# nbip/IWAE

Hardware: AMD Instinct MI355X
Metric: images/sec (train step) IWAE k=50 batch 1024 @1/2/4/8 GPU; test LLH@k=5000 (higher is better)
Workload: dtype bf16; 1 GPU; 1-layer IWAE k=50 batch 1024 per GPU (BASELINE configs[1]; N=8 is configs[4]), objective iwae_elbo, train step = forward + backward + Adam(eps=1e-4); config_id=c1, global_batch=1024, n_samples=50, parallelism=dp1, rccl_ranks=0, settle_steps=100, full=False

## Files before the change

iwae_amd/csrc/kernels.h:

```cpp
#pragma once
#include <hip/hip_runtime.h>
#include <stdint.h>

namespace iwae {

#define IWAE_DENSE_G1_DEFAULT 29u
enum { EPI_TANH = 0, EPI_HEAD = 1, EPI_DX = 2, EPI_F32 = 3, EPI_BERN = 4, EPI_SIGMOID = 5 };
enum { OBJ_VAE_ELBO = 0, OBJ_IWAE_ELBO = 1, OBJ_IWAE_EQ14 = 2, OBJ_VAE_ELBO_KL = 3, OBJ_DREG = 4 };
enum { PB_LME = 0, PB_MEAN, PB_EQ14, PB_KL, PB_PX, PB_T1, PB_T2, PB_DREG, PB_COUNT };
enum { SC_VAE_ELBO = 0, SC_VAE_ELBO_KL, SC_IWAE_ELBO, SC_IWAE_EQ14, SC_INFERENCE_LOSS, SC_MEAN_LPXZ, SC_MEAN_T1, SC_MEAN_T2, SC_KL, SC_COUNT = 16 };

struct EpsSrc {
    const float* user = nullptr;
    const float* cache = nullptr;
    int ldC = 0;
    int B = 0;
    uint64_t seed = 0;
    uint64_t row_offset = 0;
    uint32_t step = 0;
    uint32_t stream = 0;
    int k_total = 0, s_off = 0, kc = 0;
};

struct LseArgs {
// ... 4 lines not shown
    const float* head; int ldH, D, Dp;
    float* logw; float* wn; float* gx; float4* cf; float* per_b;
    int n_px_part; size_t px_stride;
    float* term0_out;
    int lme_only;
    float* gx_local; int gx_r0, gx_n;
};

struct DenseArgs {
    const uint16_t* X; int ldX;
    const char* img;
    int split;
    int M, KT, MG, mg_per_block;
    int stage_all;
    unsigned g1_mask;
    int Np32;
    uint16_t* YP; int ldYP;
    float* YF; int ldYF;
    const uint16_t* ACT; int ldACT;
    const uint16_t* XB; int ldXB; int k; int B; int Xdim;
    const float* zhead; int ldZH;
    const float* zeps; int zldE; int zD, zDp;
    uint16_t* ZPout;
    float* zlp; float* zlq;
    float* zlq_dreg;
    float* lpxz; size_t lpxz_stride;
    float* logits_out;
    int pipe;
    const char* pre_img1; int pre_KT1;
    const char* pre_img2;
    const uint16_t* pre_Z;
    uint16_t *pre_G1, *pre_G2;
    unsigned long long* stamps;
    int lse_on;
    LseArgs lse;
    uint16_t* G2W; int g2w_feat;
    int dbg;
};

struct SampleArgs {
    const float* head; int ldH; int Dp; int D; int head_per_row;
    int M, Mp, k, B;
    EpsSrc eps;
    uint16_t* ZP;
    float* ZF; int ldZF;
    const float* prior_head;
    const float* cond; int C;
    float* lp_prior; float* lq; float* lq_dreg;
};

struct BlockFwdArgs {
    const uint16_t* X; int ldX;
    const float* Xf; int Xdim; uint16_t* XPout;
    const char *img0, *img1, *img2;
    int KT0, KT1;
    int NT1, NT2;
    int R;
    uint16_t *H1, *H2; int ldH;
    float* YF; int ldYF; int split;
    int sample; SampleArgs S;
    const char* oimg; int oXdim, oH;
    const uint16_t* oXB; int oldXB; int ok;
    uint16_t* oSP; int oldS; float* olpxz;
};
struct DecBwdRowsArgs {
    const uint16_t* SP; int ldS; int KTX;
// ... 343 lines not shown
```

iwae_amd/csrc/kernels.hip:

```cpp
#include <hip/hip_runtime.h>
#include <hip/hip_ext.h>
#include <stdint.h>
#include <string.h>
#include <type_traits>
#include <algorithm>
#include "kernels.h"
#include "layout.h"

#ifdef IWAE_DIAG
#define WG_DBG(a, bit) (((a).dbg & (bit)) != 0)
#else
#define WG_DBG(a, bit) false
#endif
namespace iwae {

typedef __attribute__((ext_vector_type(8))) __bf16 bf16x8_t;
typedef __attribute__((ext_vector_type(2))) __bf16 bf16x2_t;
typedef __attribute__((ext_vector_type(4))) float f32x4;

#define LOG2PI_F 1.8378770664093453f

__device__ __forceinline__ uint32_t pack2(float a, float b) {
    bf16x2_t v;
    v[0] = (__bf16)a;
// ... 160 lines not shown
template <bool MASKED, bool KEEP>
__device__ __forceinline__ float bern8(const f32x4& a0, const f32x4& a1, const uint4& xb, int f0, int Xdim, uint4& sp) {
    float s_xl = 0.0f, s_al = 0.0f, prod = 1.0f, sv[8];
#pragma unroll
    for (int j = 0; j < 8; ++j) {
        const float l = (j < 4) ? a0[j & 3] : a1[j & 3];
        const float xm = bf_at(xb, j) - 0.5f;
        const float ope = 1.0f + exp2_raw(-fabsf(l * LOG2E_F));
        const bool in = !MASKED || (f0 + 16 * (j >> 2) + (j & 3) < Xdim);
        prod *= in ? ope : 1.0f;
        s_al += fabsf(l);
        s_xl = fmaf(xm, l, s_xl);
        if (KEEP) {
            const float h = __builtin_copysignf(rcp_fast(ope) - 0.5f, l);
            sv[j] = in ? xm - h : 0.0f;
        }
    }
    if (KEEP) sp = make_uint4(pack2(sv[0], sv[1]), pack2(sv[2], sv[3]), pack2(sv[4], sv[5]), pack2(sv[6], sv[7]));
    return s_xl - 0.5f * s_al - LN2_F * log2_raw(prod);
}

#define DENSE_UNIT 33792

#ifdef IWAE_DENSE_STAMPS
#define DS_STAMP(slot)                                                                 \
    {                                                                                  \
        unsigned long long t_;                                                         \
        __builtin_amdgcn_sched_barrier(0);                                             \
        asm volatile("s_memtime %0\n\ts_waitcnt lgkmcnt(0)" : "=s"(t_)::"memory");     \
        __builtin_amdgcn_sched_barrier(0);                                             \
        ds_sum[slot] += t_ - ds_prev;                                                  \
        ds_prev = t_;                                                                  \
    }
#else
#define DS_STAMP(slot)
#endif

template <int EPI, int KTC, int G, int NWV = (G == 2 ? 4 : 8), bool ZIN = false>
__global__ __launch_bounds__(64 * NWV, G == 1 ? 4 : ((EPI == EPI_BERN && KTC > 0) ? 2 : 1)) void dense_kernel(DenseArgs a) {
#ifdef IWAE_DENSE_STAMPS
    unsigned long long ds_sum[8] = {0, 0, 0, 0, 0, 0, 0, 0}, ds_prev = 0;
    asm volatile("s_memtime %0\n\ts_waitcnt lgkmcnt(0)" : "=s"(ds_prev)::"memory");
#endif
    extern __shared__ __attribute__((aligned(1024))) char smem[];
    const int lane = threadIdx.x & 63, wave = __builtin_amdgcn_readfirstlane(threadIdx.x >> 6);
    const int rho = lane & 15, q = lane >> 4;
    const int r0 = (blockIdx.x * NWV + wave) * (16 * G);
    int row[G], rowc[G];
    bool valid[G];
#pragma unroll
    for (int g = 0; g < G; ++g) { row[g] = r0 + G * rho + g; valid[g] = row[g] < a.M; rowc[g] = min(row[g], a.M - 1); }
    const int a_off = rho * 64 + ((q ^ hperm(rho >> 2)) * 16);
    const int KT = KTC ? KTC : a.KT;
    const int nkw = KTC ? 1 : ((KT + 7) >> 3);
    const int mg0 = blockIdx.y * a.mg_per_block;
    const int mg1 = min(a.MG, mg0 + a.mg_per_block);
    const int nunits = (mg1 - mg0) * nkw;
    const size_t gbytes = img_mg_group_bytes(KT);
    constexpr bool kPacked = (EPI == EPI_TANH || EPI == EPI_DX);
    constexpr bool kPre = (EPI == EPI_DX || EPI == EPI_BERN);
    constexpr bool kBiasInit = (EPI == EPI_BERN) && KTC > 0;

    uint4 bfr[8][G];
    auto load_b_into = [&](int kw, uint4 (&dst)[8][G]) {
#pragma unroll
        for (int ks = 0; ks < 8; ++ks) {
#pragma unroll
            for (int g = 0; g < G; ++g) {
// ... 895 lines not shown
    if (has) {
        const uint2 v = valid ? dtanh(acc, y2, gxr) : make_uint2(0, 0);
        *(uint2*)(act1 + kso * 1024 + a_off + 8 * hh) = v;
        if (valid) *(uint2*)(a.D2P + (size_t)row * a.ldH + kso * 32 + q * 8 + 4 * hh) = v;
    }
    __syncthreads();
    acc = (f32x4){0.f, 0.f, 0.f, 0.f};
#pragma unroll
    for (int ks = 0; ks < BLOCKFWD_MAX_KT; ++ks)
        if (ks < a.KT) acc = mfma16(A2[ks], *(const uint4*)(act1 + ks * 1024 + a_off), acc);
    if (has) {
        const uint2 v = valid ? dtanh(acc, y1, 1.0f) : make_uint2(0, 0);
        *(uint2*)(act2 + kso * 1024 + a_off + 8 * hh) = v;
        if (valid) *(uint2*)(a.D1P + (size_t)row * a.ldH + kso * 32 + q * 8 + 4 * hh) = v;
    }
    __syncthreads();
    acc = (f32x4){0.f, 0.f, 0.f, 0.f};
#pragma unroll
    for (int ks = 0; ks < BLOCKFWD_MAX_KT; ++ks)
        if (ks < a.KT) acc = mfma16(A1[ks], *(const uint4*)(act2 + ks * 1024 + a_off), acc);
    if (has3 && valid) {
        const int f0 = 16 * wave + 4 * q;
        if (a.DZH) *(uint2*)(a.DZH + (size_t)row * a.ldDZ + f0) = make_uint2(pack2(acc[0], acc[1]), pack2(acc[2], acc[3]));
        else *(float4*)(a.DZ + (size_t)row * a.ldDZ + f0) = make_float4(acc[0], acc[1], acc[2], acc[3]);
    }
}

#define BERN_XIMG_MAX 5
template <int KTC, bool KEEP, bool PRE, bool QW = false>
__global__ __launch_bounds__(QW ? 1024 : 512, 4) void bern_pipe_kernel(DenseArgs a) {
#ifdef IWAE_DENSE_STAMPS
    unsigned long long ds_sum[8] = {0, 0, 0, 0, 0, 0, 0, 0}, ds_prev = 0;
    asm volatile("s_memtime %0\n\ts_waitcnt lgkmcnt(0)" : "=s"(ds_prev)::"memory");
#endif
    extern __shared__ __attribute__((aligned(1024))) char smem[];
    constexpr int NWV = QW ? 16 : 8, ROWS = QW ? 200 : 128;
    constexpr int UNIT = KTC * 4096 + 1024, NPC = 4 * KTC + 1, NIDX = (NPC + NWV - 1) / NWV, NF = 2 * KTC, P = 4;
    const int lane = threadIdx.x & 63, wave = __builtin_amdgcn_readfirstlane(threadIdx.x >> 6);
    const int rho = lane & 15, q = lane >> 4;
    const int tile = QW ? min(wave, 12) : wave;
    const int qw = QW ? wave - 12 : -1;
    const int row = blockIdx.x * ROWS + tile * 16 + rho;
    const bool valid = row < a.M && tile * 16 + rho < ROWS;
    const bool storer = qw <= 0;
    if (QW && qw >= 0) __builtin_amdgcn_s_setprio(3);
    const int rowc = min(row, a.M - 1);
    const int a_off = rho * 64 + ((q ^ hperm(rho >> 2)) * 16);
    const int H = a.Np32 >> 5;
    const size_t gbytes = img_mg_group_bytes(KTC);

    auto dma_group = [&](int g, int buf) {
#pragma unroll
        for (int idx = 0; idx < NIDX; ++idx) {
            const int p = wave + NWV * idx;
            if (p < NPC)
                glds16(a.img + (size_t)g * gbytes + (size_t)p * 1024 + lane * 16,
                       (uint32_t)__builtin_amdgcn_readfirstlane((int)(lds_addr_of(smem + buf * UNIT) + (uint32_t)p * 1024u)));
        }
    };
    constexpr int MGH = (2 * KTC + 3) / 4;
    auto dma_unit = [&](int u, int buf) {
        const char* src = a.img;
        int npc = NPC;
        if (u < MGH) { src = a.pre_img1 + (size_t)u * img_mg_group_bytes(a.pre_KT1); npc = 4 * a.pre_KT1 + 1; }
        else if (u < 2 * MGH) src = a.pre_img2 + (size_t)(u - MGH) * gbytes;
        if (WG_DBG(a, 64) && u < 2 * MGH) return;
#pragma unroll
        for (int idx = 0; idx < NIDX; ++idx) {
            const int p = wave + NWV * idx;
            if (p < npc)
                glds16(src + (size_t)p * 1024 + lane * 16,
                       (uint32_t)__builtin_amdgcn_readfirstlane((int)(lds_addr_of(smem + buf * UNIT) + (uint32_t)p * 1024u)));
        }
    };
    if constexpr (PRE) dma_unit(0, 0);
    else dma_group(0, 0);
    char* lx = smem + 2 * UNIT;
    const int blk_r0 = blockIdx.x * ROWS;
    const int b0 = blk_r0 / a.k, b1 = min(blk_r0 + ROWS - 1, a.M - 1) / a.k;
    constexpr bool ZQ = PRE && QW;
    constexpr int HZ_OFF = 2 * UNIT + 128 + 4096 + 2 * KTC * 1024 + 4096 + 1024;
    float4 ze[8];
    if constexpr (PRE) {
        if (a.zhead) {
            const float* er = a.zeps + (size_t)rowc * a.zldE;
            const int flast = a.zldE - 4;
#pragma unroll
            for (int i = 0; i < 8; ++i) ze[i] = *(const float4*)(er + min(32 * (i >> 1) + 16 * (i & 1) + 4 * q, flast));
        }
    }
    if constexpr (ZQ) {
        if (a.zhead) {
            float* hzf = (float*)(smem + HZ_OFF + (size_t)8 * a.ldXB * 4);
            const int zDp = a.zDp, c4 = zDp >> 2, nimg = b1 - b0 + 1;
            for (int o = threadIdx.x; o < nimg * 2 * c4; o += 64 * NWV) {
                const int img = o / (2 * c4), r = o - img * 2 * c4, arr = r >= c4 ? 1 : 0, c = r - arr * c4;
                const float4 v = *(const float4*)(a.zhead + (size_t)(b0 + img) * a.ldZH + arr * zDp + 4 * c);
                float w[4] = {v.x, v.y, v.z, v.w};
#pragma unroll
                for (int i = 0; i < 4; ++i) w[i] = (4 * c + i < a.zD) ? w[i] : 0.0f;
                *(float4*)(hzf + (size_t)(img * 3 + arr) * zDp + 4 * c) = make_float4(w[0], w[1], w[2], w[3]);
            }
        }
    }
    const int xchunks = (b1 - b0 + 1) * a.ldXB / 8;
    for (int o = threadIdx.x; o < xchunks; o += 64 * NWV) {
        const uint4 v = *(const uint4*)(a.XB + (size_t)b0 * a.ldXB + (size_t)o * 8);
        float4 lo, hi;
        lo.x = bflo(v.x) - 0.5f; lo.y = bfhi(v.x) - 0.5f; lo.z = bflo(v.y) - 0.5f; lo.w = bfhi(v.y) - 0.5f;
        hi.x = bflo(v.z) - 0.5f; hi.y = bfhi(v.z) - 0.5f; hi.z = bflo(v.w) - 0.5f; hi.w = bfhi(v.w) - 0.5f;
        *(float4*)(lx + (size_t)o * 32) = lo;
        *(float4*)(lx + (size_t)o * 32 + 16) = hi;
    }
    const char* lxrow = lx + (size_t)(rowc / a.k - b0) * a.ldXB * 4 + q * 32;
    uint4 bfr[KTC];
    if constexpr (!PRE) {
#pragma unroll
        for (int ks = 0; ks < KTC; ++ks) {
            const uint4 v = *(const uint4*)(a.X + (size_t)rowc * a.ldX + ks * 32 + q * 8);
            bfr[ks] = valid ? v : make_uint4(0, 0, 0, 0);
        }
    } else {
        const int KT1 = a.pre_KT1, ldZ = 32 * KT1;
        uint4 zf[4];
        if (a.zhead) {
            const int zDp = a.zDp;
            const int bimg = min(rowc / a.k, b1);
            const bool dreg = a.zlq_dreg != nullptr;
            auto logsig = [&](const float* sgp, float& s1, float& s2) {
                s1 = 0.0f; s2 = 0.0f;
                for (int d = lane; d < a.zD; d += 64) {
                    const float sg = sgp[d];
                    s1 += log2_raw(sg);
                    if (dreg) s2 += log2_raw(sg + 1e-6f);
                }
                s1 = LN2_F * wave_sum(s1); s2 = LN2_F * wave_sum(s2);
            };
            float hs1 = 0.0f, hs2 = 0.0f;
            const float* hm;
            if constexpr (ZQ) {
                float* hzf = (float*)(smem + HZ_OFF + (size_t)8 * a.ldXB * 4);
                float* hsum = hzf + 8 * 3 * zDp;
                __syncthreads();
                if (wave <= b1 - b0) {
                    float s1, s2;
                    logsig(hzf + (size_t)(wave * 3 + 1) * zDp, s1, s2);
                    if (lane == 0) { hsum[2 * wave] = s1; hsum[2 * wave + 1] = s2; }
                }
                __syncthreads();
                hm = hzf + (size_t)(bimg - b0) * 3 * zDp;
                hs1 = hsum[2 * (bimg - b0)]; hs2 = hsum[2 * (bimg - b0) + 1];
            } else {
                hm = a.zhead + (size_t)bimg * a.ldZH;
                const int ilo = __builtin_amdgcn_readlane(bimg, 0), ihi = __builtin_amdgcn_readlane(bimg, 15);
                float s1, s2;
                logsig(a.zhead + (size_t)ilo * a.ldZH + zDp, s1, s2);
                hs1 = s1; hs2 = s2;
                if (ihi != ilo) {
                    logsig(a.zhead + (size_t)ihi * a.ldZH + zDp, s1, s2);
                    if (bimg != ilo) { hs1 = s1; hs2 = s2; }
                }
            }
            float sz = 0.0f, se = 0.0f, su = 0.0f;
#pragma unroll
            for (int ks = 0; ks < 4; ++ks) {
                zf[ks] = make_uint4(0, 0, 0, 0);
                if (ks < KT1) {
                    float z8[8];
#pragma unroll
                    for (int h = 0; h < 2; ++h) {
                        const int f0 = 32 * ks + 16 * h + 4 * q;
                        const float4 mu4 = *(const float4*)(hm + f0), sg4 = *(const float4*)(hm + zDp + f0);
                        const float4 e4 = ze[2 * ks + h];
                        float ev[4] = {e4.x, e4.y, e4.z, e4.w}, muv[4] = {mu4.x, mu4.y, mu4.z, mu4.w};
                        const float sgv[4] = {sg4.x, sg4.y, sg4.z, sg4.w};
                        if (32 * ks + 16 * h + 16 > a.zD) {
#pragma unroll
                            for (int i = 0; i < 4; ++i) { const bool in = f0 + i < a.zD; ev[i] = in ? ev[i] : 0.0f; muv[i] = in ? muv[i] : 0.0f; }
                        }
#pragma unroll
                        for (int i = 0; i < 4; ++i) {
                            const float z = fmaf(sgv[i], ev[i], muv[i]);
                            sz = fmaf(z, z, sz);
                            se = fmaf(ev[i], ev[i], se);
                            z8[4 * h + i] = z;
                        }
                        if (dreg) {
#pragma unroll
                            for (int i = 0; i < 4; ++i) {
                                const float u2 = (sgv[i] * __builtin_amdgcn_rcpf(sgv[i] + 1e-6f)) * ev[i];
                                su = fmaf(u2, u2, su);
                            }
                        }
                    }
                    const uint4 frag = make_uint4(pack2(z8[0], z8[1]), pack2(z8[2], z8[3]), pack2(z8[4], z8[5]), pack2(z8[6], z8[7]));
                    zf[ks] = valid ? frag : make_uint4(0, 0, 0, 0);
                    if (valid && storer && a.ZPout) *(uint4*)(a.ZPout + (size_t)row * ldZ + ks * 32 + q * 8) = frag;
                }
            }
            sz += __shfl_xor(sz, 16); sz += __shfl_xor(sz, 32);
            se += __shfl_xor(se, 16); se += __shfl_xor(se, 32);
            su += __shfl_xor(su, 16); su += __shfl_xor(su, 32);
            const float cD = 0.5f * LOG2PI_F * (float)a.zD;
            const float lp = -0.5f * sz - cD, lq = -0.5f * se - cD - hs1, lq2 = -0.5f * su - cD - hs2;
            if (q == 0 && valid && storer) { a.zlp[row] = lp; a.zlq[row] = lq; if (dreg) a.zlq_dreg[row] = lq2; }
            if constexpr (QW) {
                if (a.lse_on && q == 0 && storer) {
                    float* lz = (float*)(smem + 2 * UNIT + (size_t)8 * a.ldXB * 4 + 128 + 4096 + 2 * KTC * 1024);
                    lz[tile * 16 + rho] = lp; lz[208 + tile * 16 + rho] = lq; lz[416 + tile * 16 + rho] = lq2;
                }
            }
        } else {
#pragma unroll
            for (int ks = 0; ks < 4; ++ks) {
                zf[ks] = make_uint4(0, 0, 0, 0);
                if (ks < KT1) {
                    const uint4 v = *(const uint4*)(a.pre_Z + (size_t)rowc * ldZ + ks * 32 + q * 8);
                    zf[ks] = valid ? v : make_uint4(0, 0, 0, 0);
                }
            }
        }
        uint4 g1f[KTC];
        auto store_group = [&](uint16_t* Gout, const uint4 (&bout)[KTC], int mg) {
            if (!(valid && storer && Gout) || (QW && qw >= 0)) return;
#pragma unroll
            for (int p2 = 0; p2 < 2; ++p2)
                if (2 * mg + p2 < KTC) *(uint4*)(Gout + (size_t)row * (32 * KTC) + (2 * mg + p2) * 32 + q * 8) = bout[2 * mg + p2];
        };
        auto hidden = [&](auto nb_tag, uint4* bin, auto KTin, int ubase, uint4 (&bout)[KTC], uint16_t* Gout, const char* xch_in, char* xch_out, auto&& first) {
            constexpr int NB = decltype(nb_tag)::value;
            const bool quarter = QW && qw >= 0;
#pragma unroll
            for (int mg = 0; mg < MGH; ++mg) {
                const int u = ubase + mg, buf = u & 1;
                wait_all_vmem();
                __syncthreads();
                dma_unit(u + 1, buf ^ 1);
                if (mg == 0) first(); else store_group(Gout, bout, mg - 1);
                const char* lb = smem + buf * UNIT + a_off;
                const char* lbias = smem + buf * UNIT + KTin * 4096 + q * 16;
                if (quarter) {
                    if (mg == 0 && xch_in) {
#pragma unroll
                        for (int ks = 0; ks < NB; ++ks) bin[ks] = *(const uint4*)(xch_in + ks * 1024 + lane * 16);
                    }
                    const float4 c = *(const float4*)(lbias + 64 * qw);
                    f32x4 acc1 = (f32x4){c.x, c.y, c.z, c.w};
#pragma unroll
                    for (int ks = 0; ks < NB; ++ks)
                        if (ks < KTin) acc1 = mfma16(*(const uint4*)(lb + (ks * 4 + qw) * 1024), bin[ks], acc1);
                    const int ft = 4 * mg + qw, kso = ft >> 1, hh = ft & 1;
                    if (kso < KTC) {
                        const uint2 piece = make_uint2(pack2(tanh_fast(acc1[0]), tanh_fast(acc1[1])), pack2(tanh_fast(acc1[2]), tanh_fast(acc1[3])));
                        *(uint2*)(xch_out + kso * 1024 + lane * 16 + 8 * hh) = valid ? piece : make_uint2(0, 0);
                        if (valid && Gout) *(uint2*)(Gout + (size_t)row * (32 * KTC) + kso * 32 + q * 8 + 4 * hh) = piece;
                    }
                    continue;
                }
                f32x4 acc[4];
#pragma unroll
                for (int t = 0; t < 4; ++t) {
                    const float4 c = *(const float4*)(lbias + 64 * t);
                    acc[t] = (f32x4){c.x, c.y, c.z, c.w};
                }
                lds_pipeline<NB * 4, 4>(
                    [&](int i) { return (i >> 2) < KTin ? *(const uint4*)(lb + i * 1024) : make_uint4(0, 0, 0, 0); },
                    [&](int i, const uint4& av) { if ((i >> 2) < KTin) acc[i & 3] = mfma16(av, bin[i >> 2], acc[i & 3]); });
#pragma unroll
                for (int p2 = 0; p2 < 2; ++p2) {
                    const int kso = 2 * mg + p2;
                    if (kso < KTC) {
                        float v[8];
#pragma unroll
                        for (int j = 0; j < 8; ++j) v[j] = tanh_fast(acc[2 * p2 + (j >> 2)][j & 3]);
                        const uint4 frag = make_uint4(pack2(v[0], v[1]), pack2(v[2], v[3]), pack2(v[4], v[5]), pack2(v[6], v[7]));
                        bout[kso] = frag;
                    }
                }
            }
        };
        char* xch1 = smem + 2 * UNIT + (size_t)8 * a.ldXB * 4 + 128 + 4096;
        char* xch2 = xch1 + KTC * 1024;
        DS_STAMP(0);
        if (WG_DBG(a, 128)) { wait_all_vmem(); return; }
        if (KT1 == 4) hidden(std::integral_constant<int, 4>{}, zf, std::integral_constant<int, 4>{}, 0, g1f, a.pre_G1, nullptr, xch1, [] {});
        else hidden(std::integral_constant<int, 4>{}, zf, KT1, 0, g1f, a.pre_G1, nullptr, xch1, [] {});
        DS_STAMP(1);
        if (WG_DBG(a, 512)) { wait_all_vmem(); return; }
        hidden(std::integral_constant<int, KTC>{}, g1f, std::integral_constant<int, KTC>{}, MGH, bfr, a.pre_G2, xch1, xch2, [&] { store_group(a.pre_G1, g1f, MGH - 1); });
        DS_STAMP(2);
        if (WG_DBG(a, 256)) { wait_all_vmem(); return; }
    }

    f32x4 accA[2], accB[2];
    uint4 st[2];
    float rowacc = 0.0f;
    auto store_s = [&](int h, const uint4& v) {
        if (KEEP && valid && !WG_DBG(a, 32)) *(uint4*)(a.YP + (size_t)row * a.ldYP + 32 * h + 8 * q) = v;
    };
    auto stage = [&](auto masked, auto domfma, f32x4 (&accC)[2], f32x4 (&accN)[2], int h, int bufN, int tbN, float4 (&xq)[2], float4 (&xnx)[2], uint4& sp) {
        constexpr bool MASKED = decltype(masked)::value, MF = decltype(domfma)::value;
        const char* lb = smem + bufN * UNIT + a_off + tbN * 1024;
        uint4 av[P];
        if constexpr (MF) {
            const char* lbias = smem + bufN * UNIT + KTC * 4096 + tbN * 64 + q * 16;
            const float4 c0 = *(const float4*)lbias, c1 = *(const float4*)(lbias + 64);
            accN[0] = (f32x4){c0.x, c0.y, c0.z, c0.w};
            accN[1] = (f32x4){c1.x, c1.y, c1.z, c1.w};
#pragma unroll
            for (int i = 0; i < P; ++i) av[i] = *(const uint4*)(lb + ((i >> 1) * 4 + (i & 1)) * 1024);
        }
        float s_xl = 0.0f, s_al = 0.0f, prod = 1.0f, sv[8] = {0.f, 0.f, 0.f, 0.f, 0.f, 0.f, 0.f, 0.f};
        const int f0 = 32 * h + 4 * q;
        asm volatile("" : "+v"(xq[0].x), "+v"(xq[0].y), "+v"(xq[0].z), "+v"(xq[0].w), "+v"(xq[1].x), "+v"(xq[1].y), "+v"(xq[1].z), "+v"(xq[1].w));
        const float xm8[8] = {xq[0].x, xq[0].y, xq[0].z, xq[0].w, xq[1].x, xq[1].y, xq[1].z, xq[1].w};
        xnx[0] = *(const float4*)(lxrow + (h + 1) * 128); xnx[1] = *(const float4*)(lxrow + (h + 1) * 128 + 16);
#pragma unroll
        for (int c = 0; c < 4; ++c) {
            if (MF && c > 0) asm volatile("" : "+v"(accC[0]), "+v"(accC[1]), "+v"(prod), "+v"(s_al), "+v"(s_xl), "+v"(accN[0]), "+v"(accN[1]));
            else asm volatile("" : "+v"(accC[0]), "+v"(accC[1]), "+v"(prod), "+v"(s_al), "+v"(s_xl));
            const float l0 = (c < 2) ? accC[0][(2 * c) & 3] : accC[1][(2 * c) & 3];
            const float l1 = (c < 2) ? accC[0][(2 * c + 1) & 3] : accC[1][(2 * c + 1) & 3];
// ... 135 lines not shown
    DS_STAMP(4);
    for (; h < H; ++h) {
        const int nh = h + 1, bufN = (nh >> 1) & 1, tbN = (nh & 1) * 2;
        const bool domf = nh < H;
        if (h & 1) boundary(h, domf);
        if (!fullw) {
            if ((h & 1) && q_real(h >> 1)) q_stage(h >> 1, domf && q_real((h >> 1) + 1));
            continue;
        }
        uint4 sp = make_uint4(0, 0, 0, 0);
        if (domf) stage(std::true_type{}, std::true_type{}, accA, accB, h, bufN, tbN, xbq, xbr, sp);
        else stage(std::true_type{}, std::false_type{}, accA, accB, h, bufN, tbN, xbq, xbr, sp);
        accA[0] = accB[0]; accA[1] = accB[1];
        xbq[0] = xbr[0]; xbq[1] = xbr[1];
        if (h & 1) st[1] = sp; else st[0] = sp;
    }
    if (fullw) {
        if (H & 1) { if (H >= 2) store_s(H - 2, st[1]); store_s(H - 1, st[0]); }
        else store_s(H - 1, st[1]);
    } else if ((H & 1) && q_real((H - 1) >> 1)) {
        q_stage((H - 1) >> 1, false);
    }

    DS_STAMP(5);
    float v = rowacc;
    v += __shfl_xor(v, 16);
    v += __shfl_xor(v, 32);
#ifdef IWAE_DENSE_STAMPS
    if (a.stamps && lane == 0) {
        unsigned long long t_;
        asm volatile("s_memtime %0\n\ts_waitcnt lgkmcnt(0)" : "=s"(t_)::"memory");
        ds_sum[6] = t_ - ds_prev;
        for (int i = 0; i < 8; ++i) a.stamps[((size_t)blockIdx.x * NWV + wave) * 8 + i] = ds_sum[i];
    }
#endif
    if constexpr (QW) {
        __syncthreads();
        float* part = (float*)smem;
        if (qw >= 0 && q == 0) part[qw * 16 + rho] = v;
        __syncthreads();
        if (qw == 0) v = part[rho] + part[16 + rho] + part[32 + rho] + part[48 + rho];
        if (qw > 0 && !(PRE && a.lse_on)) return;
    }
    if (q == 0 && valid && storer) a.lpxz[row] = v;
    if constexpr (QW && PRE) {
        if (a.lse_on) {
            float* lz = (float*)(smem + 2 * UNIT + (size_t)8 * a.ldXB * 4 + 128 + 4096 + 2 * KTC * 1024);
            if (q == 0 && storer) lz[624 + tile * 16 + rho] = v;
            __syncthreads();
            const int nimg = ROWS / a.k, b = blockIdx.x * nimg + wave;
            if (wave < nimg && b < a.B) {
                struct Src {
                    const float* lz; int l0; bool made_z, made_lqd;
                    __device__ __forceinline__ float px(const LseArgs&, int s, int) const { return lz[624 + l0 + s]; }
                    __device__ __forceinline__ float px_total(const LseArgs&, int s, int) const { return lz[624 + l0 + s]; }
                    __device__ __forceinline__ float term(const LseArgs& la, int t, int s, int r) const {
                        return (made_z && t == 1) ? lz[l0 + s] : (made_z && t == 2) ? lz[208 + l0 + s] : la.term[t][r];
                    }
                    __device__ __forceinline__ float lq_dreg(const LseArgs& la, int s, int r) const { return made_lqd ? lz[416 + l0 + s] : la.lq_dreg[r]; }
                };
                LseArgs la = a.lse;
                la.gx_local = lz + 832; la.gx_r0 = blockIdx.x * ROWS; la.gx_n = ROWS;
                lse_image(la, b, lane, Src{lz, wave * a.k, a.zhead != nullptr, a.zhead != nullptr && a.zlq_dreg != nullptr});
            }
            if (a.G2W) {
                __syncthreads();
// ... 2731 lines not shown
```

iwae_amd/csrc/model.hip:

```cpp
#include <hip/hip_runtime.h>
#include <math.h>
#include <stdio.h>
#include <string.h>
#include <stddef.h>
#include <stdlib.h>
#include <string>
#include <vector>
#include <algorithm>
#include <random>
#include <memory>
#include <dlfcn.h>
#include <rccl/rccl.h>
#include "../../include/iwae_amd.h"
#include "kernels.h"
#include "layout.h"

using namespace iwae;

static_assert(sizeof(iwae_config) == 64 && offsetof(iwae_config, struct_size) == 0 && offsetof(iwae_config, seed) == 32 && offsetof(iwae_config, cond_dim) == 48 &&
              offsetof(iwae_config, cond_prior) == 52 && offsetof(iwae_config, precision) == 56, "iwae_config layout is part of the ABI (iwae_amd/_capi.py)");
static_assert(sizeof(iwae_scalars) == 64 && sizeof(iwae_tensors) == 12 * sizeof(void*), "ABI struct layout");

static thread_local std::string g_err;
static int fail(int code, const std::string& msg) { g_err = msg; return code; }
// ... 426 lines not shown
            m->ev_start[id].push_back(a); m->ev_stop[id].push_back(b);
        }
        (void)hipEventRecord(m->ev_start[id][m->ev_used[id]], ts);
    }
    ~ScopedTimer() {
        if (!on) return;
        (void)hipEventRecord(m->ev_stop[id][m->ev_used[id]], ts);
        m->ev_used[id] += 1;
    }
};

static inline int eps_ld(const iwae_model* m, int layer) { return 4 * ((m->D[layer] + 3) / 4); }
EpsSrc eps_src(iwae_model* m, int layer) {
    EpsSrc e;
    e.user = nullptr;
    e.cache = m->epsc_ptr[layer];
    e.ldC = eps_ld(m, layer);
    if (m->user_eps) e.user = ptr<float>(m->epsbuf) + (layer == 0 ? 0 : (size_t)m->k * m->B * m->D[0]);
    e.B = m->B;
    e.seed = m->cfg.seed;
    e.row_offset = (uint64_t)m->call.batch_offset * (uint64_t)m->k;
    e.step = m->noise_step;
    e.stream = (uint32_t)layer;
    if (m->call.k_total > 0) {
        e.k_total = m->call.k_total; e.s_off = m->call.s_off; e.kc = m->k;
        e.row_offset = (uint64_t)m->call.batch_offset * (uint64_t)m->call.k_total;
    }
    return e;
}

int attach_dense_stamps(iwae_model* m, int epi, DenseArgs& a) {
    if (m->dstamp_epi != epi || m->dstamp_kt != a.KT || (a.M < 4096 && a.KT <= 8)) return IWAE_OK;
    m->dstamp_waves = std::max(((a.M + 127) / 128) * ((a.MG + a.mg_per_block - 1) / a.mg_per_block) * 4, epi == EPI_BERN ? ((a.M + 127) / 128) * 16 : 0);
    CHK(ensure(m->dstamps, (size_t)m->dstamp_waves * 64, m->stream));
    a.stamps = ptr<unsigned long long>(m->dstamps);
    return IWAE_OK;
}

int join_side(iwae_model* m) {
    if (m->dec2_pending) {
        HIPCHK(hipStreamWaitEvent(m->stream, m->ev_dec2, 0));
        m->dec2_pending = false;
    }
    if (!m->dec_pending) return IWAE_OK;
    HIPCHK(hipStreamWaitEvent(m->stream, m->ev_dec, 0));
    m->dec_pending = false;
    return IWAE_OK;
}

int dense_fwd(iwae_model* m, Linear& L, int epi, const uint16_t* XP, int rows, uint16_t* YP, float* YF, int ldYF, const SampleArgs* zin = nullptr) {
    DenseArgs a;
    memset(&a, 0, sizeof(a));
    a.X = XP; a.ldX = L.Kp32; a.img = L.imgF;
    a.split = (L.nsub == 2) ? L.joff[1] : (1 << 30);
    a.M = rows; a.KT = L.KT; a.MG = L.MG; a.mg_per_block = (rows <= 8192) ? 1 : L.MG; a.Np32 = L.Np32; a.g1_mask = m->dense_g1_mask;
    a.stage_all = (a.mg_per_block == 1 && L.KT > 8 && (L.KT + 7) / 8 <= 4) ? 1 : 0;
    if (zin) {
        a.zhead = zin->head; a.ldZH = zin->ldH; a.zeps = zin->eps.cache; a.zldE = zin->eps.ldC; a.zD = zin->D; a.zDp = zin->Dp;
        a.ZPout = zin->ZP; a.zlp = zin->lp_prior; a.zlq = zin->lq; a.k = zin->k;
        a.mg_per_block = L.MG;
    }
    a.YP = YP; a.ldYP = L.Np32; a.YF = YF; a.ldYF = ldYF;
    CHK(attach_dense_stamps(m, epi, a));
    launch_dense(epi, a, m->stream);
    HIPCHK(hipGetLastError());
    return IWAE_OK;
}

// ... 2669 lines not shown
        {"dec.g1", 0, &m->wdec1.g1P, M, H0, Hp0},
        {"dec.g2", 0, &m->wdec1.g2P, M, H0, Hp0},
        {"dec.dl", 0, &m->wdec1.dlP, M, m->X, m->Xp32},
        {"dec.d2", 0, &m->wdec1.d2P, M, H0, Hp0},
        {"dec.d1", 0, &m->wdec1.d1P, M, H0, Hp0},
        {"dec.dz", 2, &m->wdec1.dz, M, Dp0, Dp0},
        {"gx", 2, &m->gx, M, 1, 1}, {"wn", 2, &m->wn, M, 1, 1}, {"log_w", 2, &m->logw, M, 1, 1},
    };
    if (m->cfg.n_layers == 2) {
        const int H1 = m->H[1], Hp1 = m->Hp[1], D1 = m->D[1], Dp1 = m->Dp[1];
        std::vector<Ent> e2 = {
            {"enc2.h1", 0, &m->wenc2.h1P, M, H1, Hp1}, {"enc2.h2", 0, &m->wenc2.h2P, M, H1, Hp1},
            {"enc2.head", 2, &m->wenc2.head, M, 2 * Dp1, 2 * Dp1}, {"enc2.dhead", 0, &m->wenc2.dheadP, M, 2 * Dp1, 2 * Dp1},
            {"enc2.dx", 2, &m->wenc2.dx, M, Dp0, Dp0},
            {"z2", 0, &m->zP[1], M, D1, Dp1},
            {"dec2.h1", 0, &m->wdec2.h1P, M, H1, Hp1}, {"dec2.h2", 0, &m->wdec2.h2P, M, H1, Hp1},
            {"dec2.head", 2, &m->wdec2.head, M, 2 * Dp0, 2 * Dp0}, {"dec2.dhead", 0, &m->wdec2.dheadP, M, 2 * Dp0, 2 * Dp0},
            {"dec2.dx", 2, &m->wdec2.dx, M, Dp1, Dp1},
            {"dz1_direct", 2, &m->dzdir, M, Dp0, Dp0},
        };
        ents.insert(ents.end(), e2.begin(), e2.end());
    }
    if (strcmp(name, "dense_stamps") == 0) {
        if (rows) *rows = m->dstamp_waves;
        if (cols) *cols = 8;
        if (!out) return IWAE_OK;
        if (!m->dstamps.p) return fail(IWAE_ERR_STATE, "dense stamps not enabled (STAMPS=1 build + options dense_stamps_epi / dense_stamps_kt)");
        std::vector<unsigned long long> h((size_t)m->dstamp_waves * 8);
        HIPCHK(hipStreamSynchronize(m->stream));
        HIPCHK(hipMemcpy(h.data(), m->dstamps.p, h.size() * 8, hipMemcpyDeviceToHost));
        for (size_t i = 0; i < h.size(); ++i) out[i] = (float)h[i];
        return IWAE_OK;
    }
    if (strcmp(name, "stamps") == 0) {
        const int nw = (Mp / 64) * 4;
        if (rows) *rows = nw;
        if (cols) *cols = 8;
        if (!out) return IWAE_OK;
        if (!m->stamps.p) return fail(IWAE_ERR_STATE, "stamps not enabled (DIAG=1 build + option stamps)");
        std::vector<unsigned long long> h((size_t)nw * 8);
        HIPCHK(hipStreamSynchronize(m->stream));
        HIPCHK(hipMemcpy(h.data(), m->stamps.p, h.size() * 8, hipMemcpyDeviceToHost));
        for (size_t i = 0; i < h.size(); ++i) out[i] = (float)h[i];
        return IWAE_OK;
    }
    for (const Ent& e : ents) {
        if (strcmp(e.nm, name) != 0) continue;
        if (rows) *rows = e.R;
        if (cols) *cols = e.F;
        if (!out) return IWAE_OK;
        if (!e.buf->p) return fail(IWAE_ERR_STATE, std::string("debug_tensor: buffer not populated: ") + name);
        const size_t n = (size_t)e.R * e.F;
        if (cap < n) return fail(IWAE_ERR_ARG, "debug_tensor: output too small");
        if (e.kind == 2) {
            HIPCHK(hipMemcpyAsync(out, e.buf->p, n * 4, hipMemcpyDefault, m->stream));
        } else {
            CHK(ensure(m->scratch, n * 4, m->stream));
            launch_unpack_p(ptr<uint16_t>(*e.buf), e.R, e.F, e.Fp, ptr<float>(m->scratch), m->stream);
            HIPCHK(hipMemcpyAsync(out, m->scratch.p, n * 4, hipMemcpyDefault, m->stream));
        }
        HIPCHK(hipStreamSynchronize(m->stream));
        return IWAE_OK;
    }
    return fail(IWAE_ERR_ARG, std::string("debug_tensor: unknown name ") + name);
}

// ... 2 lines not shown
```

Before: 5.260 million images/s.

## Overlap prologue loads with first weight DMA in bern pipe kernel

In the pre-fused Bernoulli pipeline kernel, the prologue now issues the first two weight-unit DMAs up front. It also issues the z-head, sigma and X loads before any waiting, so their latencies overlap instead of being serialized. The first hidden-layer iteration skips its initial vmem wait and barrier, and the Z/logprob stores and X staging are deferred into the first-iteration callback. This trims the prologue's serialized global-memory round trips, at the cost of more live registers, more complex barrier ordering, and new sub-stamp timing instrumentation (compiled only in stamps builds).

```diff
diff --git a/iwae_amd/csrc/kernels.h b/iwae_amd/csrc/kernels.h
--- a/iwae_amd/csrc/kernels.h
+++ b/iwae_amd/csrc/kernels.h
@@ -60,6 +60,7 @@
     const uint16_t* pre_Z;
     uint16_t *pre_G1, *pre_G2;
     unsigned long long* stamps;
+    unsigned* stamps_sub;
     int lse_on;
     LseArgs lse;
     uint16_t* G2W; int g2w_feat;
diff --git a/iwae_amd/csrc/kernels.hip b/iwae_amd/csrc/kernels.hip
--- a/iwae_amd/csrc/kernels.hip
+++ b/iwae_amd/csrc/kernels.hip
@@ -216,8 +216,25 @@
         ds_sum[slot] += t_ - ds_prev;                                                  \
         ds_prev = t_;                                                                  \
     }
+#define DS_SUB_MARK()                                                                  \
+    {                                                                                  \
+        __builtin_amdgcn_sched_barrier(0);                                             \
+        asm volatile("s_memtime %0\n\ts_waitcnt lgkmcnt(0)" : "=s"(ds_sprev)::"memory"); \
+        __builtin_amdgcn_sched_barrier(0);                                             \
+    }
+#define DS_SUB(slot)                                                                   \
+    {                                                                                  \
+        unsigned long long t_;                                                         \
+        __builtin_amdgcn_sched_barrier(0);                                             \
+        asm volatile("s_memtime %0\n\ts_waitcnt lgkmcnt(0)" : "=s"(t_)::"memory");     \
+        __builtin_amdgcn_sched_barrier(0);                                             \
+        ds_sub[slot] += (unsigned)(t_ - ds_sprev);                                     \
+        ds_sprev = t_;                                                                 \
+    }
 #else
 #define DS_STAMP(slot)
+#define DS_SUB_MARK()
+#define DS_SUB(slot)
 #endif
 
 template <int EPI, int KTC, int G, int NWV = (G == 2 ? 4 : 8), bool ZIN = false>
@@ -1179,6 +1196,8 @@
 #ifdef IWAE_DENSE_STAMPS
     unsigned long long ds_sum[8] = {0, 0, 0, 0, 0, 0, 0, 0}, ds_prev = 0;
     asm volatile("s_memtime %0\n\ts_waitcnt lgkmcnt(0)" : "=s"(ds_prev)::"memory");
+    unsigned ds_sub[24] = {0, 0, 0, 0, 0, 0, 0, 0, 0, 0, 0, 0, 0, 0, 0, 0, 0, 0, 0, 0, 0, 0, 0, 0};
+    unsigned long long ds_sprev = ds_prev;
 #endif
     extern __shared__ __attribute__((aligned(1024))) char smem[];
     constexpr int NWV = QW ? 16 : 8, ROWS = QW ? 200 : 128;
@@ -1220,7 +1239,7 @@
                        (uint32_t)__builtin_amdgcn_readfirstlane((int)(lds_addr_of(smem + buf * UNIT) + (uint32_t)p * 1024u)));
         }
     };
-    if constexpr (PRE) dma_unit(0, 0);
+    if constexpr (PRE) { dma_unit(0, 0); dma_unit(1, 1); }
     else dma_group(0, 0);
     char* lx = smem + 2 * UNIT;
     const int blk_r0 = blockIdx.x * ROWS;
@@ -1228,37 +1247,74 @@
     constexpr bool ZQ = PRE && QW;
     constexpr int HZ_OFF = 2 * UNIT + 128 + 4096 + 2 * KTC * 1024 + 4096 + 1024;
     float4 ze[8];
+    float4 hv0 = make_float4(0.0f, 0.0f, 0.0f, 0.0f);
+    float sgl[4] = {1.0f, 1.0f, 1.0f, 1.0f};
+    int bimg = 0, ilo = 0, ihi = 0;
+    const int nhead = (ZQ && a.zhead) ? (b1 - b0 + 1) * 2 * (a.zDp >> 2) : 0;
+    auto head_piece = [&](int o, int& dst, int& c) -> const float* {
+        const int c4 = a.zDp >> 2, img = o / (2 * c4), r = o - img * 2 * c4, arr = r >= c4 ? 1 : 0;
+        c = r - arr * c4;
+        dst = (img * 3 + arr) * a.zDp + 4 * c;
+        return a.zhead + (size_t)(b0 + img) * a.ldZH + arr * a.zDp + 4 * c;
+    };
     if constexpr (PRE) {
         if (a.zhead) {
             const float* er = a.zeps + (size_t)rowc * a.zldE;
             const int flast = a.zldE - 4;
 #pragma unroll
             for (int i = 0; i < 8; ++i) ze[i] = *(const float4*)(er + min(32 * (i >> 1) + 16 * (i & 1) + 4 * q, flast));
-        }
-    }
+            bimg = min(rowc / a.k, b1);
+            auto sig_req = [&](int img, int j) {
+                const float* sgp = a.zhead + (size_t)img * a.ldZH + a.zDp;
+#pragma unroll
+                for (int t = 0; t < 2; ++t)
+                    if (lane + 64 * t < a.zD) sgl[j + t] = sgp[lane + 64 * t];
+            };
+            if constexpr (ZQ) {
+                int dst, c;
+                if ((int)threadIdx.x < nhead) hv0 = *(const float4*)head_piece(threadIdx.x, dst, c);
+                if (wave <= b1 - b0) sig_req(b0 + wave, 0);
+            } else {
+                ilo = __builtin_amdgcn_readlane(bimg, 0); ihi = __builtin_amdgcn_readlane(bimg, 15);
+                sig_req(ilo, 0);
+                if (ihi != ilo) sig_req(ihi, 2);
+            }
+        }
+    }
+    const int xchunks = (b1 - b0 + 1) * a.ldXB / 8;
+    uint4 xv0 = make_uint4(0, 0, 0, 0);
+    if ((int)threadIdx.x < xchunks) xv0 = *(const uint4*)(a.XB + (size_t)b0 * a.ldXB + (size_t)threadIdx.x * 8);
+    DS_SUB(0);
     if constexpr (ZQ) {
         if (a.zhead) {
+            wait_all_vmem();
+            DS_SUB(1);
             float* hzf = (float*)(smem + HZ_OFF + (size_t)8 * a.ldXB * 4);
-            const int zDp = a.zDp, c4 = zDp >> 2, nimg = b1 - b0 + 1;
-            for (int o = threadIdx.x; o < nimg * 2 * c4; o += 64 * NWV) {
-                const int img = o / (2 * c4), r = o - img * 2 * c4, arr = r >= c4 ? 1 : 0, c = r - arr * c4;
-                const float4 v = *(const float4*)(a.zhead + (size_t)(b0 + img) * a.ldZH + arr * zDp + 4 * c);
+            auto put_head = [&](int dst, int c, const float4& v) {
                 float w[4] = {v.x, v.y, v.z, v.w};
 #pragma unroll
                 for (int i = 0; i < 4; ++i) w[i] = (4 * c + i < a.zD) ? w[i] : 0.0f;
-                *(float4*)(hzf + (size_t)(img * 3 + arr) * zDp + 4 * c) = make_float4(w[0], w[1], w[2], w[3]);
-            }
-        }
-    }
-    const int xchunks = (b1 - b0 + 1) * a.ldXB / 8;
-    for (int o = threadIdx.x; o < xchunks; o += 64 * NWV) {
-        const uint4 v = *(const uint4*)(a.XB + (size_t)b0 * a.ldXB + (size_t)o * 8);
-        float4 lo, hi;
-        lo.x = bflo(v.x) - 0.5f; lo.y = bfhi(v.x) - 0.5f; lo.z = bflo(v.y) - 0.5f; lo.w = bfhi(v.y) - 0.5f;
-        hi.x = bflo(v.z) - 0.5f; hi.y = bfhi(v.z) - 0.5f; hi.z = bflo(v.w) - 0.5f; hi.w = bfhi(v.w) - 0.5f;
-        *(float4*)(lx + (size_t)o * 32) = lo;
-        *(float4*)(lx + (size_t)o * 32 + 16) = hi;
-    }
+                *(float4*)(hzf + dst) = make_float4(w[0], w[1], w[2], w[3]);
+            };
+            int dst, c;
+            if ((int)threadIdx.x < nhead) { head_piece(threadIdx.x, dst, c); put_head(dst, c, hv0); }
+            for (int o = threadIdx.x + 64 * NWV; o < nhead; o += 64 * NWV) {
+                const float4 v = *(const float4*)head_piece(o, dst, c);
+                put_head(dst, c, v);
+            }
+        }
+    }
+    auto stage_x = [&]() {
+        auto put_x = [&](int o, const uint4& v) {
+            float4 lo, hi;
+            lo.x = bflo(v.x) - 0.5f; lo.y = bfhi(v.x) - 0.5f; lo.z = bflo(v.y) - 0.5f; lo.w = bfhi(v.y) - 0.5f;
+            hi.x = bflo(v.z) - 0.5f; hi.y = bfhi(v.z) - 0.5f; hi.z = bflo(v.w) - 0.5f; hi.w = bfhi(v.w) - 0.5f;
+            *(float4*)(lx + (size_t)o * 32) = lo;
+            *(float4*)(lx + (size_t)o * 32 + 16) = hi;
+        };
+        if ((int)threadIdx.x < xchunks) put_x(threadIdx.x, xv0);
+        for (int o = threadIdx.x + 64 * NWV; o < xchunks; o += 64 * NWV) put_x(o, *(const uint4*)(a.XB + (size_t)b0 * a.ldXB + (size_t)o * 8));
+    };
     const char* lxrow = lx + (size_t)(rowc / a.k - b0) * a.ldXB * 4 + q * 32;
     uint4 bfr[KTC];
     if constexpr (!PRE) {
@@ -1267,19 +1323,23 @@
             const uint4 v = *(const uint4*)(a.X + (size_t)rowc * a.ldX + ks * 32 + q * 8);
             bfr[ks] = valid ? v : make_uint4(0, 0, 0, 0);
         }
+        stage_x();
     } else {
         const int KT1 = a.pre_KT1, ldZ = 32 * KT1;
         uint4 zf[4];
+        const bool dreg = a.zlq_dreg != nullptr;
+        float lp = 0.0f, lq = 0.0f, lq2 = 0.0f;
         if (a.zhead) {
             const int zDp = a.zDp;
-            const int bimg = min(rowc / a.k, b1);
-            const bool dreg = a.zlq_dreg != nullptr;
-            auto logsig = [&](const float* sgp, float& s1, float& s2) {
+            auto logsig = [&](const float* sg2, float& s1, float& s2) {
                 s1 = 0.0f; s2 = 0.0f;
-                for (int d = lane; d < a.zD; d += 64) {
-                    const float sg = sgp[d];
-                    s1 += log2_raw(sg);
-                    if (dreg) s2 += log2_raw(sg + 1e-6f);
+#pragma unroll
+                for (int t = 0; t < 2; ++t) {
+                    if (lane + 64 * t < a.zD) {
+                        const float sg = sg2[t];
+                        s1 += log2_raw(sg);
+                        if (dreg) s2 += log2_raw(sg + 1e-6f);
+                    }
                 }
                 s1 = LN2_F * wave_sum(s1); s2 = LN2_F * wave_sum(s2);
             };
@@ -1288,23 +1348,22 @@
             if constexpr (ZQ) {
                 float* hzf = (float*)(smem + HZ_OFF + (size_t)8 * a.ldXB * 4);
                 float* hsum = hzf + 8 * 3 * zDp;
-                __syncthreads();
                 if (wave <= b1 - b0) {
                     float s1, s2;
-                    logsig(hzf + (size_t)(wave * 3 + 1) * zDp, s1, s2);
+                    logsig(sgl, s1, s2);
                     if (lane == 0) { hsum[2 * wave] = s1; hsum[2 * wave + 1] = s2; }
                 }
                 __syncthreads();
+                DS_SUB(2);
                 hm = hzf + (size_t)(bimg - b0) * 3 * zDp;
                 hs1 = hsum[2 * (bimg - b0)]; hs2 = hsum[2 * (bimg - b0) + 1];
             } else {
                 hm = a.zhead + (size_t)bimg * a.ldZH;
-                const int ilo = __builtin_amdgcn_readlane(bimg, 0), ihi = __builtin_amdgcn_readlane(bimg, 15);
                 float s1, s2;
-                logsig(a.zhead + (size_t)ilo * a.ldZH + zDp, s1, s2);
+                logsig(sgl, s1, s2);
                 hs1 = s1; hs2 = s2;
                 if (ihi != ilo) {
-                    logsig(a.zhead + (size_t)ihi * a.ldZH + zDp, s1, s2);
+                    logsig(sgl + 2, s1, s2);
                     if (bimg != ilo) { hs1 = s1; hs2 = s2; }
                 }
             }
@@ -1342,15 +1401,13 @@
                     }
                     const uint4 frag = make_uint4(pack2(z8[0], z8[1]), pack2(z8[2], z8[3]), pack2(z8[4], z8[5]), pack2(z8[6], z8[7]));
                     zf[ks] = valid ? frag : make_uint4(0, 0, 0, 0);
-                    if (valid && storer && a.ZPout) *(uint4*)(a.ZPout + (size_t)row * ldZ + ks * 32 + q * 8) = frag;
                 }
             }
             sz += __shfl_xor(sz, 16); sz += __shfl_xor(sz, 32);
             se += __shfl_xor(se, 16); se += __shfl_xor(se, 32);
             su += __shfl_xor(su, 16); su += __shfl_xor(su, 32);
             const float cD = 0.5f * LOG2PI_F * (float)a.zD;
-            const float lp = -0.5f * sz - cD, lq = -0.5f * se - cD - hs1, lq2 = -0.5f * su - cD - hs2;
-            if (q == 0 && valid && storer) { a.zlp[row] = lp; a.zlq[row] = lq; if (dreg) a.zlq_dreg[row] = lq2; }
+            lp = -0.5f * sz - cD; lq = -0.5f * se - cD - hs1; lq2 = -0.5f * su - cD - hs2;
             if constexpr (QW) {
                 if (a.lse_on && q == 0 && storer) {
                     float* lz = (float*)(smem + 2 * UNIT + (size_t)8 * a.ldXB * 4 + 128 + 4096 + 2 * KTC * 1024);
@@ -1367,6 +1424,15 @@
                 }
             }
         }
+        auto z_out = [&]() {
+            if (!(a.zhead && valid && storer)) return;
+            if (a.ZPout) {
+#pragma unroll
+                for (int ks = 0; ks < 4; ++ks)
+                    if (ks < KT1) *(uint4*)(a.ZPout + (size_t)row * ldZ + ks * 32 + q * 8) = zf[ks];
+            }
+            if (q == 0) { a.zlp[row] = lp; a.zlq[row] = lq; if (dreg) a.zlq_dreg[row] = lq2; }
+        };
         uint4 g1f[KTC];
         auto store_group = [&](uint16_t* Gout, const uint4 (&bout)[KTC], int mg) {
             if (!(valid && storer && Gout) || (QW && qw >= 0)) return;
@@ -1374,15 +1440,20 @@
             for (int p2 = 0; p2 < 2; ++p2)
                 if (2 * mg + p2 < KTC) *(uint4*)(Gout + (size_t)row * (32 * KTC) + (2 * mg + p2) * 32 + q * 8) = bout[2 * mg + p2];
         };
-        auto hidden = [&](auto nb_tag, uint4* bin, auto KTin, int ubase, uint4 (&bout)[KTC], uint16_t* Gout, const char* xch_in, char* xch_out, auto&& first) {
+        auto hidden = [&](auto nb_tag, uint4* bin, auto KTin, int ubase, bool lead, bool open0, uint4 (&bout)[KTC], uint16_t* Gout, const char* xch_in, char* xch_out, auto&& first) {
             constexpr int NB = decltype(nb_tag)::value;
             const bool quarter = QW && qw >= 0;
 #pragma unroll
             for (int mg = 0; mg < MGH; ++mg) {
                 const int u = ubase + mg, buf = u & 1;
-                wait_all_vmem();
-                __syncthreads();
-                dma_unit(u + 1, buf ^ 1);
+                if (!(mg == 0 && open0)) {
+                    DS_SUB_MARK();
+                    wait_all_vmem();
+                    DS_SUB(6 + 2 * u);
+                    __syncthreads();
+                    DS_SUB(7 + 2 * u);
+                }
+                if (!(mg == 0 && lead)) dma_unit(u + 1, buf ^ 1);
                 if (mg == 0) first(); else store_group(Gout, bout, mg - 1);
                 const char* lb = smem + buf * UNIT + a_off;
                 const char* lbias = smem + buf * UNIT + KTin * 4096 + q * 16;
@@ -1428,13 +1499,21 @@
         };
         char* xch1 = smem + 2 * UNIT + (size_t)8 * a.ldXB * 4 + 128 + 4096;
         char* xch2 = xch1 + KTC * 1024;
+        DS_SUB(3);
         DS_STAMP(0);
-        if (WG_DBG(a, 128)) { wait_all_vmem(); return; }
-        if (KT1 == 4) hidden(std::integral_constant<int, 4>{}, zf, std::integral_constant<int, 4>{}, 0, g1f, a.pre_G1, nullptr, xch1, [] {});
-        else hidden(std::integral_constant<int, 4>{}, zf, KT1, 0, g1f, a.pre_G1, nullptr, xch1, [] {});
+        if (WG_DBG(a, 128)) { z_out(); wait_all_vmem(); return; }
+        const bool open0 = ZQ && a.zhead;
+        auto first1 = [&] {
+            DS_SUB_MARK();
+            z_out();
+            stage_x();
+            DS_SUB(4);
+        };
+        if (KT1 == 4) hidden(std::integral_constant<int, 4>{}, zf, std::integral_constant<int, 4>{}, 0, true, open0, g1f, a.pre_G1, nullptr, xch1, first1);
+        else hidden(std::integral_constant<int, 4>{}, zf, KT1, 0, true, open0, g1f, a.pre_G1, nullptr, xch1, first1);
         DS_STAMP(1);
         if (WG_DBG(a, 512)) { wait_all_vmem(); return; }
-        hidden(std::integral_constant<int, KTC>{}, g1f, std::integral_constant<int, KTC>{}, MGH, bfr, a.pre_G2, xch1, xch2, [&] { store_group(a.pre_G1, g1f, MGH - 1); });
+        hidden(std::integral_constant<int, KTC>{}, g1f, std::integral_constant<int, KTC>{}, MGH, false, false, bfr, a.pre_G2, xch1, xch2, [&] { store_group(a.pre_G1, g1f, MGH - 1); });
         DS_STAMP(2);
         if (WG_DBG(a, 256)) { wait_all_vmem(); return; }
     }
@@ -1636,6 +1715,8 @@
         asm volatile("s_memtime %0\n\ts_waitcnt lgkmcnt(0)" : "=s"(t_)::"memory");
         ds_sum[6] = t_ - ds_prev;
         for (int i = 0; i < 8; ++i) a.stamps[((size_t)blockIdx.x * NWV + wave) * 8 + i] = ds_sum[i];
+        if (a.stamps_sub)
+            for (int i = 0; i < 24; ++i) a.stamps_sub[((size_t)blockIdx.x * NWV + wave) * 24 + i] = ds_sub[i];
     }
 #endif
     if constexpr (QW) {
diff --git a/iwae_amd/csrc/model.hip b/iwae_amd/csrc/model.hip
--- a/iwae_amd/csrc/model.hip
+++ b/iwae_amd/csrc/model.hip
@@ -482,8 +482,9 @@
 int attach_dense_stamps(iwae_model* m, int epi, DenseArgs& a) {
     if (m->dstamp_epi != epi || m->dstamp_kt != a.KT || (a.M < 4096 && a.KT <= 8)) return IWAE_OK;
     m->dstamp_waves = std::max(((a.M + 127) / 128) * ((a.MG + a.mg_per_block - 1) / a.mg_per_block) * 4, epi == EPI_BERN ? ((a.M + 127) / 128) * 16 : 0);
-    CHK(ensure(m->dstamps, (size_t)m->dstamp_waves * 64, m->stream));
+    CHK(ensure(m->dstamps, (size_t)m->dstamp_waves * (64 + 96), m->stream));
     a.stamps = ptr<unsigned long long>(m->dstamps);
+    a.stamps_sub = epi == EPI_BERN ? (unsigned*)(a.stamps + (size_t)m->dstamp_waves * 8) : nullptr;
     return IWAE_OK;
 }
 
@@ -3219,6 +3220,17 @@
         for (size_t i = 0; i < h.size(); ++i) out[i] = (float)h[i];
         return IWAE_OK;
     }
+    if (strcmp(name, "dense_stamps_sub") == 0) {
+        if (rows) *rows = m->dstamp_waves;
+        if (cols) *cols = 24;
+        if (!out) return IWAE_OK;
+        if (!m->dstamps.p) return fail(IWAE_ERR_STATE, "dense stamps not enabled (STAMPS=1 build + options dense_stamps_epi / dense_stamps_kt)");
+        std::vector<unsigned> h((size_t)m->dstamp_waves * 24);
+        HIPCHK(hipStreamSynchronize(m->stream));
+        HIPCHK(hipMemcpy(h.data(), (const char*)m->dstamps.p + (size_t)m->dstamp_waves * 64, h.size() * 4, hipMemcpyDeviceToHost));
+        for (size_t i = 0; i < h.size(); ++i) out[i] = (float)h[i];
+        return IWAE_OK;
+    }
     if (strcmp(name, "stamps") == 0) {
         const int nw = (Mp / 64) * 4;
         if (rows) *rows = nw;
```

Measured after the change: 5.270 million images/s (median of 3 runs). No clear change (+0.2%).
